# pavlidic/Binary-SpGEMM

Hardware: AMD Instinct MI355X
Metric: output nnz/sec (GNZ/s) (higher is better)
Workload: dtype int32; 1 GPU; R-MAT scale 22, edge factor 16, (a,b,c,d)=(0.30,0.25,0.25,0.20), seed 1, A*A; n=4194304, nnz_a=67108664, products=1336443900, nnz_c=1336366087, parallelism=row-shards x1 cut at equal work, B replicated, priming_steps=0, flow=auto, full=False

## Files before the change

binary-spgemm_amd/bspgemm/__init__.py:

```python
import ctypes as C
import os
import subprocess
import weakref

import numpy as np

os.environ.setdefault("OMP_NUM_THREADS", str(min(16, len(os.sched_getaffinity(0)))))
os.environ.setdefault("GPU_MAX_HW_QUEUES", "8")

_PKG = os.path.dirname(os.path.abspath(__file__))
_ROOT = os.path.dirname(_PKG)
LIB_PATH = os.path.join(_ROOT, "libbspgemm.so")

_I32P = np.ctypeslib.ndpointer(dtype=np.int32, flags="C_CONTIGUOUS")
_I64P = np.ctypeslib.ndpointer(dtype=np.int64, flags="C_CONTIGUOUS")

STATUS = {0: "OK", 1: "ERR_INVALID", 2: "ERR_ALLOC", 3: "ERR_HIP", 4: "ERR_NO_DEVICE",
          5: "ERR_OVERFLOW", 6: "ERR_IO", 7: "ERR_FORMAT", 8: "ERR_COMM", 9: "ERR_SIZE"}

EXPORTS = [
    "bspgemm_status_string", "bspgemm_last_error", "bspgemm_create", "bspgemm_destroy",
    "bspgemm_set_stream", "bspgemm_synchronize", "bspgemm_matrix_upload", "bspgemm_matrix_wrap_device",
    "bspgemm_matrix_free", "bspgemm_matrix_rows", "bspgemm_matrix_cols", "bspgemm_matrix_nnz",
    "bspgemm_multiply", "bspgemm_multiply_masked", "bspgemm_multiply_masked_ex", "bspgemm_result_rows", "bspgemm_result_nnz",
# ... 20 lines not shown
    def __init__(self, status, where=""):
        self.status = status
        msg = lib().bspgemm_last_error().decode(errors="replace") if _lib is not None else ""
        super().__init__("%s: %s %s" % (where, STATUS.get(status, status), msg))


MAX_BINS = 20
FLOWS = {"auto": 0, "upper-bound": 1, "exact": 2}
MASK_COMPLEMENT = 1
CLOSURE_TRANSITIVE = 1
SELECT_OPS = {"tril": 1, "triu": 2, "offdiag": 3}
SETOPS = {"or": 1, "and": 2, "andnot": 3, "xor": 4}
SYMMETRIZE_DROP_DIAGONAL = 1
COMPARES = {">=": 1, ">": 2, "<=": 3, "<": 4, "==": 5, "!=": 6}
OPTIONS = {"class_streams": 1, "blocked_extents": 2, "check": 3, "small_path": 4, "padded_rows": 5,
           "shared_slots": 6}


class Stats(C.Structure):
    _fields_ = [("rows", C.c_int64), ("nnz_a", C.c_int64), ("products", C.c_int64), ("nnz_c", C.c_int64),
                ("bytes_alg", C.c_int64), ("bytes_read_alg", C.c_int64), ("rows_per_bin", C.c_int64 * MAX_BINS),
                ("ms_total", C.c_float), ("ms_symbolic", C.c_float), ("ms_prepass", C.c_float),
                ("ms_count", C.c_float), ("ms_numeric", C.c_float), ("ms_stitch", C.c_float),
                ("ms_bin", C.c_float * MAX_BINS), ("ms_bin_count", C.c_float * MAX_BINS),
                ("t_bin", C.c_float * MAX_BINS), ("t_bin_count", C.c_float * MAX_BINS), ("bins", C.c_int),
                ("bin_cap", C.c_int * MAX_BINS), ("flow", C.c_int), ("prepass_kernel", C.c_int),
                ("class_streams", C.c_int), ("small_path", C.c_int), ("checked", C.c_int), ("padded_rows", C.c_int)]

    def as_dict(self):
        arrays = ("rows_per_bin", "ms_bin", "ms_bin_count", "t_bin", "t_bin_count", "bin_cap")
        d = {k: getattr(self, k) for k, _ in self._fields_ if k not in arrays}
# ... 527 lines not shown
```

binary-spgemm_amd/csrc/context.hip:

```cpp
#include "internal.hpp"

using namespace bsp;

thread_local char bspgemm_err_text[512] = "";

extern "C" const char *bspgemm_last_error(void) { return g_err; }

extern "C" const char *bspgemm_status_string(bspgemm_status s)
{
    switch (s) {
    case BSPGEMM_OK: return "ok";
    case BSPGEMM_ERR_INVALID: return "invalid argument";
    case BSPGEMM_ERR_ALLOC: return "allocation failed";
    case BSPGEMM_ERR_HIP: return "HIP runtime error";
    case BSPGEMM_ERR_NO_DEVICE: return "no gfx950 device (this library has no CPU fallback)";
    case BSPGEMM_ERR_OVERFLOW: return "result exceeds the int32 drop-in interface";
    case BSPGEMM_ERR_IO: return "file I/O error";
    case BSPGEMM_ERR_FORMAT: return "Matrix Market banner rejected";
    case BSPGEMM_ERR_SIZE: return "Matrix Market size line or entry rejected";
    case BSPGEMM_ERR_COMM: return "RCCL error";
    }
    return "unknown status";
}

// ... 121 lines not shown
        for (auto &ph : sl.ev_cls) for (auto &c : ph) for (auto &e : c) HIPCHK_B(hipEventCreate(&e));
    }
    HIPCHK_B(hipStreamCreateWithFlags(&ctx->stream_b, hipStreamNonBlocking));
    HIPCHK_B(hipStreamCreateWithFlags(&ctx->stream_c, hipStreamNonBlocking));
    HIPCHK_B(hipEventCreateWithFlags(&ctx->ev_join, hipEventDisableTiming));
    for (auto &t : ctx->ev_tile) for (auto &e : t) HIPCHK_B(hipEventCreateWithFlags(&e, hipEventDisableTiming));
    ctx->cache_budget = prop.totalGlobalMem / 4;
    if (const char *e = getenv("BSPGEMM_FLOW"))
        ctx->flow = !strcmp(e, "exact") ? BSPGEMM_FLOW_EXACT : (!strcmp(e, "upper-bound") || !strcmp(e, "ub")) ? BSPGEMM_FLOW_UPPER_BOUND : BSPGEMM_FLOW_AUTO;
    if (const char *e = getenv("BSPGEMM_CLASS_TIMING")) ctx->class_timing = atoi(e) != 0;
    if (const char *e = getenv("BSPGEMM_CLASS_STREAMS")) { const int n = atoi(e); ctx->class_streams = n < 1 ? 1 : (n > 3 ? 3 : n); }
    ctx->check = getenv("BSPGEMM_CHECK") != nullptr;
    if (const char *e = getenv("BSPGEMM_RW_BLK")) ctx->rw_blk = atoi(e) ? 1 : 0;
    if (const char *e = getenv("BSPGEMM_SMALL")) ctx->small = atoi(e) ? 1 : 0;
    if (const char *e = getenv("BSPGEMM_PAD_ROWS")) { const int v = atoi(e); ctx->pad_rows = v < 0 ? -1 : (v ? 1 : 0); }
    if (const char *e = getenv("BSPGEMM_SHARED_SLOTS")) { const int v = atoi(e); ctx->shared_slots = v < 0 ? -1 : (v > kSharedSlotsMax ? kSharedSlotsMax : v); }
    ctx->debug_alloc = getenv("BSPGEMM_DEBUG_ALLOC") != nullptr;
    ctx->dropin_timing = getenv("BSPGEMM_DROPIN_TIMING") != nullptr;
    if (ctx->debug_alloc)
        fprintf(stderr, "[bspgemm] device %d: %s, %zu MiB, %d CUs; result cache budget %zu MiB\n", device,
                prop.gcnArchName, (size_t)(prop.totalGlobalMem >> 20), prop.multiProcessorCount, ctx->cache_budget >> 20);
    *out = ctx;
    return BSPGEMM_OK;
}

extern "C" void bspgemm_destroy(bspgemm_context *ctx)
{
    if (!ctx) return;
    hipSetDevice(ctx->device);
    if (ctx->stream) hipStreamSynchronize(ctx->stream);
// ... 379 lines not shown
    case BSPGEMM_OPT_CHECK:
        ctx->check = value != 0;
        return BSPGEMM_OK;
    case BSPGEMM_OPT_SMALL_PATH:
        if (value < -1 || value > 1) return FAIL(BSPGEMM_ERR_INVALID, "small path: -1, 0 or 1");
        ctx->small = value;
        return BSPGEMM_OK;
    case BSPGEMM_OPT_PADDED_ROWS:
        if (value < -1 || value > 1) return FAIL(BSPGEMM_ERR_INVALID, "padded rows: -1, 0 or 1");
        ctx->pad_rows = value;
        return BSPGEMM_OK;
    case BSPGEMM_OPT_SHARED_SLOTS:
        if (value < -1) return FAIL(BSPGEMM_ERR_INVALID, "shared slots: -1, 0 or a count");
        ctx->shared_slots = value > kSharedSlotsMax ? kSharedSlotsMax : value;
        return BSPGEMM_OK;
    }
    return FAIL(BSPGEMM_ERR_INVALID, "unknown option");
}

extern "C" int bspgemm_get_option(const bspgemm_context *ctx, bspgemm_option opt)
{
    if (!ctx) return INT_MIN;
    switch (opt) {
    case BSPGEMM_OPT_CLASS_STREAMS: return ctx->class_streams;
    case BSPGEMM_OPT_BLOCKED_EXTENTS: return ctx->rw_blk;
    case BSPGEMM_OPT_CHECK: return ctx->check ? 1 : 0;
    case BSPGEMM_OPT_SMALL_PATH: return ctx->small;
    case BSPGEMM_OPT_PADDED_ROWS: return ctx->pad_rows;
    case BSPGEMM_OPT_SHARED_SLOTS: return ctx->shared_slots;
    }
    return INT_MIN;
}

extern "C" int bspgemm_matrix_uses_padded_rows(const bspgemm_matrix *m)
{
    if (!m || m->pad_state == 0) return -1;
    return m->pad_state == 1 ? 1 : 0;
}

extern "C" int bspgemm_matrix_uses_blocked_table(const bspgemm_matrix *m)
{
    if (!m || m->blk16_state == 0) return -1;
    return m->blk16_state == 1 ? 1 : 0;
}
// ... 66 lines not shown
```

binary-spgemm_amd/csrc/internal.hpp:

```cpp
#pragma once
#include "../../include/bspgemm.h"
#include "kernels.hpp"

#include <hip/hip_runtime.h>

#include <climits>
#include <cstdio>
#include <cstdlib>
#include <cstring>
#include <chrono>
#include <new>

extern thread_local char bspgemm_err_text[512];
#define g_err bspgemm_err_text

static inline bspgemm_status fail(bspgemm_status st, const char *what, const char *file, int line)
{
    snprintf(g_err, sizeof g_err, "%s (%s:%d)", what, file, line);
    return st;
}
#define FAIL(st, what) fail((st), (what), __FILE__, __LINE__)
#define HIPCHK(call)                                                                       \
    do {                                                                                   \
        hipError_t e_ = (call);                                                            \
// ... 74 lines not shown
    bsp::SmallTiles *d_small_tiles = nullptr;
    unsigned *d_err = nullptr;
    int *chunk_row = nullptr;
    size_t chunk_cap = 0;
    HostScalars *h = nullptr;
    struct CachedBuf { void *p; size_t bytes; };
    CachedBuf cache[8] = {};
    size_t cache_budget = 0;
    int flow = BSPGEMM_FLOW_AUTO;
    bool class_timing = false;
    int class_streams = 2;
    bool check = false;
    int rw_blk = -1;
    int pad_rows = 0;
    int small = -1;
    int shared_slots = -1;
    bool debug_alloc = false;
    bool dropin_timing = false;
};

extern "C" int bspgemm_par_max_plus_one(const int *idx, long long n);
extern "C" void bspgemm_par_prefault(void *p, size_t bytes);
extern "C" long long bspgemm_par_output_bound(const int *Acol, const int *Arow, int r0, int r1, const int *Brow, int brows, long long cap);

struct bspgemm_matrix {
    bspgemm_context *ctx;
    int rows, cols;
    long long nnz;
    int *d_row_ptr, *d_col_idx;
    bool owned;
// ... 42 lines not shown
```

binary-spgemm_amd/csrc/kernels.hpp:

```cpp
#pragma once
#include <hip/hip_runtime.h>
#include <stdint.h>
#include <stdlib.h>

namespace bsp {

enum class MaskMode { None, Keep, Drop, Insert, Count };

constexpr int kWaveBins = 16;
constexpr int kNumBins = kWaveBins + 4;
constexpr int kRankBin = kWaveBins + 1;
constexpr int kMidBin = kWaveBins + 2;
constexpr int kDenseBin = kWaveBins + 3;
constexpr int kRankCap = 6144;
int rank_cap_for_cols(long long cols);
constexpr int kMaxBins = 20;
constexpr int kWaveChunks[kWaveBins + 1] = {0, 1, 2, 3, 4, 5, 6, 7, 8, 10, 12, 14, 16, 20, 24, 28, 32};
constexpr int kMaxWaveCap = 64 * kWaveChunks[kWaveBins];
constexpr int kMidCap = 524288;
inline int mid_cap_for_cols(long long cols)
{
    const long long passes = (cols + (1ll << 18) - 1) >> 18;
    if (passes <= 1) return kMidCap;
    const long long c = kMidCap / passes;
// ... 44 lines not shown
    int bin_count[kNumBins];
    unsigned long long max_f;
};
void launch_scan_and_bin(const long long *F, int n, int row_begin, const int *Arow, long long *prefix,
                         long long *partials, int *bin_tiles, int *bin_count, RowRec *rec,
                         long long *recpre, int *cnt, int heavy_cols, long long *hpartials, int mid_cap, int rank_cap, int bound_cols,
                         hipStream_t s, PrepScalars *scal = nullptr, const long long *true_F = nullptr);

constexpr int kCompactGran = 4096;
inline size_t compact_chunk_rows(long long max_out) { return (size_t)((max_out + kCompactGran - 1) / kCompactGran) + 2; }
void launch_scan_counts(const int *cnt, int n, long long *prefix, long long *partials,
                        const long long *base, hipStream_t s, int *chunk_row = nullptr);

constexpr int kSharedSlotsMax = 16;
int wave_shared_max(int bin, int shared_slots);
constexpr unsigned kErrCapacity = 1u;
constexpr unsigned kErrStaleTable = 2u;
hipError_t launch_wave_rows(int bin, int levels, const int2 *ab, const int *Bcol, int cols,
                            const RowRec *rec, const long long *recpre, const long long *row_ptr, int nrows,
                            int row_begin, int *tmp, int *cnt, unsigned *err, MaskMode mode, const int *Frow, const int *Fcol,
                            hipStream_t s, bool count_only = false, int shared_slots = 0);
void launch_check_tables(const int *row_ptr, int rows, const unsigned char *deg8, const int *blk16, const int *pad_ptr, unsigned *err,
                         hipStream_t s);

void launch_place_heavy(const int *tmp, const RowRec *rec, const long long *recpre, int nrows,
                        const long long *row_ptr, int row_begin, int *col_idx, hipStream_t s);

hipError_t launch_dense_rows(int bin, const int2 *ab, const int *Bcol, long long nnzB, int cols,
                             const RowRec *rec, const long long *recpre, int nrows, int row_begin,
                             int *tmp, int *cnt, MaskMode mode, const int *Frow, const int *Fcol, hipStream_t s,
                             int *vals = nullptr);

constexpr int kHeavySortMax = 8192;
void launch_order_heavy(const RowRec *rec, const long long *recpre, int n, RowRec *rec_out, long long *pre_out, hipStream_t s);

bool wave_masked_supported(int cols);
void launch_wave_masked(int bin, const int2 *ab, const int *Bcol, int cols, const int *Frow, const int *Fcol,
                        const RowRec *rec, const long long *recpre, int nrows, int row_begin,
                        int *tmp, int *cnt, int *vals, hipStream_t s);
hipError_t launch_class(int bin, const int2 *ab, const int *Bcol, long long nnzB, int cols, const RowRec *rec,
                        const long long *recpre, int nrows, int row_begin, int *tmp, int *cnt, unsigned *err, MaskMode mode,
                        const int *Frow, const int *Fcol, hipStream_t s, bool count_only = false, int *vals = nullptr,
                        int shared_slots = 0);
void launch_mask_lengths(const long long *F, const int *Frow, int row_begin, int n, long long *mlen, hipStream_t s);
void launch_mask_lengths_count(const long long *F, const int *Frow, int row_begin, int n, long long *mlen,
                               unsigned long long *maxF, hipStream_t s);
void launch_insert_lengths(const long long *F, const int *Drow, int row_begin, int n, long long *size, hipStream_t s);

void launch_compact(const int *tmp, const long long *Fprefix, const long long *row_ptr,
                    int row_lo, int row_hi, long long max_out, int *col_idx, hipStream_t s, const int *chunk_row = nullptr);

constexpr int kSmallMaxProducts = 65536;
constexpr int kSmallMaxRow = 2048;
constexpr int kSmallMaxRows = 1 << 17;
constexpr int kSmallMaxNnzA = 32768;
struct SmallScalars {
    long long totalF;
    long long nnzC;
// ... 42 lines not shown
```

binary-spgemm_amd/csrc/multiply.hip:

```cpp
#include "internal.hpp"

using namespace bsp;

static bspgemm_status check_operands(bspgemm_context *ctx, const bspgemm_matrix *A, const bspgemm_matrix *B,
                                     int row_begin, int row_end)
{
    if (!ctx || !A || !B) return FAIL(BSPGEMM_ERR_INVALID, "NULL operand");
    if (A->ctx != ctx || B->ctx != ctx) return FAIL(BSPGEMM_ERR_INVALID, "operand belongs to another context");
    if (row_begin < 0 || row_end < row_begin || row_end > A->rows) return FAIL(BSPGEMM_ERR_INVALID, "row range");
    if (B->rows < A->cols) return FAIL(BSPGEMM_ERR_INVALID, "B has fewer rows than A has columns");
    return BSPGEMM_OK;
}


static void class_order(const int *bin_count, long long total_products, int *order, int *lane)
{
    int light[kWaveBins];
    for (int k = 0; k < kWaveBins; k++) light[k] = k + 1;
    const long long heavy_lower_bound = ((long long)bin_count[kRankBin] + bin_count[kMidBin] + bin_count[kDenseBin]) * kMaxWaveCap;
    if (heavy_lower_bound * 8 < total_products) {
        long long key[kNumBins] = {};
        for (int b = 1; b <= kWaveBins; b++) key[b] = (long long)bin_count[b] * kWaveChunks[b];
        for (int a = 1; a < kWaveBins; a++)
            for (int c = a; c > 0 && key[light[c]] > key[light[c - 1]]; c--) {
// ... 204 lines not shown

    if (!ctx->check && result_cached(ctx, result_bytes_colidx(totalF))) {
        HIPCHK_B(alloc_col_idx(ctx, C, totalF));
    } else {
        HIPCHK_B(hipStreamSynchronize(s));
        if (h->nnzC < 0 || h->nnzC > totalF) return bail(FAIL(BSPGEMM_ERR_HIP, "symbolic pass counted more outputs than products"));
        HIPCHK_B(alloc_col_idx(ctx, C, col_cap_for(totalF, h->nnzC)));
    }

    if (R > 0) {
        const int levels = wave_levels_for_cols(B->cols);
        auto emit = [&](int b, int n, const RowRec *rec, const long long *recpre, hipStream_t sx) {
            if (b <= kWaveBins)
                return launch_wave_rows(b, levels, ctx->ab, Bcol, B->cols, rec, recpre, C->d_row_ptr, n, row_begin,
                                        C->d_col_idx, nullptr, ctx->d_err, MaskMode::None, nullptr, nullptr, sx, false,
                                        ctx->shared_slots);
            launch_place_heavy(ctx->tmp, rec, recpre, n, C->d_row_ptr, row_begin, C->d_col_idx, sx);
            return hipSuccess;
        };
        if (bspgemm_status st = class_phase(ctx, 1, totalF, cls_n[1], true, emit)) return bail(st);
    }
    HIPCHK_B(hipEventRecord(slot.ev[3], s));
    if (R > 0) {
        HIPCHK_B(hipEventRecord(ctx->ev_join, ctx->stream_c));
        HIPCHK_B(hipStreamWaitEvent(s, ctx->ev_join, 0));
    }
    return finish_flow(ctx, C, B, totalF, rank_cap_for_cols(B->cols), cls_n, out);
}


static bspgemm_status multiply_upper_bound(bspgemm_context *ctx, const bspgemm_matrix *A,
// ... 40 lines not shown
    if (count && R > 0 && h->prep.max_f > (unsigned long long)INT_MAX)
        return bail(FAIL(BSPGEMM_ERR_OVERFLOW, "a row has more than INT_MAX products: its counts may not fit int32"));
    if (bspgemm_status st = ensure_tmp(ctx, (size_t)total + 1)) return bail(st);
    if (count)
        if (bspgemm_status st = ensure_tmpv(ctx, (size_t)total + 1)) return bail(st);
    if (bspgemm_status st = ensure_chunk_rows(ctx, compact_chunk_rows(total))) return bail(st);
    if (result_cached(ctx, result_bytes_colidx(total))) HIPCHK_B(alloc_col_idx(ctx, C, total));
    HIPCHK_B(hipEventRecord(slot.ev[2], s));

    int cls_n[2][kNumBins] = {};
    if (R > 0) {
        const int *Frow = Fm ? Fm->d_row_ptr : nullptr, *Fcol = Fm ? Fm->d_col_idx : nullptr;
        auto place = [&](int b, int n, const RowRec *rec, const long long *recpre, hipStream_t sx) {
            if (!keep) hub_order(ctx, b, n, rec, recpre, sx);
            return launch_class(b, ctx->ab, Bcol, B->gather_nnz(), B->cols, rec, recpre, n, row_begin, ctx->tmp, ctx->cnt,
                                ctx->d_err, mode, Frow, Fcol, sx, false, count ? ctx->tmpv : nullptr, ctx->shared_slots);
        };
        if (bspgemm_status st = class_phase(ctx, 1, h->products, cls_n[1], false, place)) return bail(st);
        HIPCHK_B(hipEventRecord(slot.ev[3], s));
        launch_scan_counts(ctx->cnt, R, C->d_row_ptr, ctx->partials, nullptr, s, ctx->chunk_row);
    } else {
        HIPCHK_B(hipMemsetAsync(C->d_row_ptr, 0, sizeof(long long), s));
        HIPCHK_B(hipEventRecord(slot.ev[3], s));
    }
    HIPCHK_B(hipMemcpyAsync(&h->nnzC, C->d_row_ptr + R, sizeof(long long), hipMemcpyDeviceToHost, s));
    if (!C->d_col_idx) {
        HIPCHK_B(hipStreamSynchronize(s));
        HIPCHK_B(alloc_col_idx(ctx, C, col_cap_for(total, h->nnzC)));
    }
    if (count)
        HIPCHK_B(result_alloc(ctx, reinterpret_cast<void **>(&C->d_values), result_bytes_colidx(C->col_cap)));
// ... 317 lines not shown
```

binary-spgemm_amd/csrc/wave_rows.hip:

```cpp
#include "kernels.hpp"

namespace bsp {

template <int LEVELS, MaskMode MODE>
void launch_wave_levels(int bin, const int2 *ab, const int *Bcol, int cols, int topw, const RowRec *rec,
                        const long long *recpre, const long long *row_ptr, int nrows, int row_begin, int *tmp, int *cnt,
                        unsigned *err, const int *Frow, const int *Fcol, hipStream_t s, bool count, int shared_max);
#define BSP_WAVE_EXTERN1(L, M) \
    extern template void launch_wave_levels<L, MaskMode::M>(int, const int2 *, const int *, int, int, const RowRec *, \
        const long long *, const long long *, int, int, int *, int *, unsigned *, const int *, const int *, hipStream_t, bool, int);
#define BSP_WAVE_EXTERN(L) BSP_WAVE_EXTERN1(L, None) BSP_WAVE_EXTERN1(L, Drop) BSP_WAVE_EXTERN1(L, Insert)
BSP_WAVE_EXTERN(1) BSP_WAVE_EXTERN(2) BSP_WAVE_EXTERN(3) BSP_WAVE_EXTERN(4) BSP_WAVE_EXTERN(5)
#undef BSP_WAVE_EXTERN
#undef BSP_WAVE_EXTERN1

static int wave_top_words(int levels, int cols)
{
    const long long span = 1ll << (5 * levels);
    return (int)(((long long)cols + span - 1) / span);
}

int wave_shared_max(int bin, int shared_slots)
{
    static_assert(kWaveBins == 16, "one entry per capacity class");
    static const int auto_max[kWaveBins + 1] = {0, 4, 4, 4, 4, 8, 8, 8, 8, 4, 4, 4, 4, 0, 0, 0, 0};
    if (bin < 1 || bin > kWaveBins || kWaveChunks[bin] > 16) return 0;
    if (shared_slots < 0) return auto_max[bin];
    return shared_slots > kSharedSlotsMax ? kSharedSlotsMax : shared_slots;
}

hipError_t launch_wave_rows(int bin, int levels, const int2 *ab, const int *Bcol, int cols,
                            const RowRec *rec, const long long *recpre, const long long *row_ptr, int nrows, int row_begin,
                            int *tmp, int *cnt, unsigned *err, MaskMode mode, const int *Frow, const int *Fcol, hipStream_t s,
                            bool count_only, int shared_slots)
{
    if (mode == MaskMode::Keep || mode == MaskMode::Count || (count_only && mode != MaskMode::None)) return hipErrorInvalidValue;
    if (nrows <= 0) return hipSuccess;
#define BSP_WAVE_ROW(M) {launch_wave_levels<1, MaskMode::M>, launch_wave_levels<2, MaskMode::M>, launch_wave_levels<3, MaskMode::M>, \
                         launch_wave_levels<4, MaskMode::M>, launch_wave_levels<5, MaskMode::M>}
    static const decltype(&launch_wave_levels<1, MaskMode::None>) by_levels[3][5] = {BSP_WAVE_ROW(None), BSP_WAVE_ROW(Drop),
                                                                                      BSP_WAVE_ROW(Insert)};
#undef BSP_WAVE_ROW
    const int m = mode == MaskMode::Drop ? 1 : (mode == MaskMode::Insert ? 2 : 0);
    by_levels[m][(levels < 5 ? levels : 5) - 1](bin, ab, Bcol, cols, wave_top_words(levels, cols), rec, recpre, row_ptr, nrows,
                                                row_begin, tmp, cnt, err, Frow, Fcol, s, count_only,
                                                count_only ? 0 : wave_shared_max(bin, shared_slots));
    return hipSuccess;
}

hipError_t launch_class(int bin, const int2 *ab, const int *Bcol, long long nnzB, int cols, const RowRec *rec,
                        const long long *recpre, int nrows, int row_begin, int *tmp, int *cnt, unsigned *err, MaskMode mode,
                        const int *Frow, const int *Fcol, hipStream_t s, bool count_only, int *vals, int shared_slots)
{
    if (bin > kWaveBins)
        return launch_dense_rows(bin, ab, Bcol, nnzB, cols, rec, recpre, nrows, row_begin, tmp, cnt, mode, Frow, Fcol, s, vals);
    if (mode != MaskMode::Keep && mode != MaskMode::Count)
        return launch_wave_rows(bin, wave_levels_for_cols(cols), ab, Bcol, cols, rec, count_only ? nullptr : recpre, nullptr,
                                nrows, row_begin, count_only ? nullptr : tmp, cnt, err, mode, Frow, Fcol, s, count_only,
                                shared_slots);
    if (!wave_masked_supported(cols))
        return launch_dense_rows(bin, ab, Bcol, nnzB, cols, rec, recpre, nrows, row_begin, tmp, cnt, mode, Frow, Fcol, s, vals);
    launch_wave_masked(bin, ab, Bcol, cols, Frow, Fcol, rec, recpre, nrows, row_begin, tmp, cnt,
                       mode == MaskMode::Count ? vals : nullptr, s);
    return hipSuccess;
}

}
```

binary-spgemm_amd/csrc/wave_rows.inc:

```
#include "kernels.hpp"
#include "wave.hpp"

namespace bsp {

constexpr int waves_per_cu(int w, int bytes) { return (w * bytes > 64 * 1024) ? 0 : (160 * 1024 / (w * bytes)) * w; }

constexpr int prev_wave_chunks(int chunks)
{
    int prev = 0;
    for (int b = 1; b <= kWaveBins; b++) {
        if (kWaveChunks[b] == chunks) return prev;
        prev = kWaveChunks[b];
    }
    return 0;
}

template <int LEVELS, int CHUNKS, int TWP>
struct WaveCfg {
    static constexpr int CAP = 64 * CHUNKS;
    static constexpr int SW = (CHUNKS <= 2) ? CHUNKS : ((CHUNKS + 3) & ~3);
    static constexpr int SLOTS = 64 * SW;
    static constexpr int TOPW = 64 * TWP;
    static constexpr int bytes_per_wave = 4 * TOPW + 2 * TOPW + 8 * CHUNKS + 4 * SLOTS
                                          + (LEVELS >= 2 ? 4 * SLOTS : 16)
                                          + (LEVELS >= 3 ? 4 * SLOTS + 2 * SLOTS : 32)
                                          + (LEVELS >= 4 ? 2 * SLOTS : 16);
    static constexpr int w4 = waves_per_cu(4, bytes_per_wave), w2 = waves_per_cu(2, bytes_per_wave);
    static constexpr int WAVES = (w4 >= w2 && w4 > 0) ? 4 : (w2 > 0 ? 2 : 1);
    static constexpr int RPW = (CHUNKS >= 16) ? kRowsPerWave / 2 : kRowsPerWave;
    static constexpr int FULL = prev_wave_chunks(CHUNKS);
};

template <int CHUNKS, bool SWZ>
__device__ __forceinline__ void store_row(int *out, int n, const u32 *stage, int lane)
{
    const __amdgpu_buffer_rsrc_t rs = __builtin_amdgcn_make_buffer_rsrc((void *)out, (short)0, n * 4, 0x00020000);
#pragma unroll
    for (int c = 0; c < CHUNKS; c++) {
        const int t = c * 64 + lane;
        __builtin_amdgcn_raw_buffer_store_b32(stage[SWZ ? stage_swz(t) : t], rs, t * 4, 0, 2);
    }
}

__device__ __forceinline__ int2 load_extent(const int2 *p)
{
    const long long v = __builtin_nontemporal_load(reinterpret_cast<const long long *>(p));
    return make_int2((int)(u32)v, (int)(u32)((u64)v >> 32));
}

constexpr int kDropBatch = 4;
template <int CHUNKS, bool SWZ>
__device__ __forceinline__ int drop_mask_cols(u32 *stage, int n, u32 *hit, const int *__restrict__ Fcol, int f0, int mlen, int lane)
{
    auto at = [](int p) { return SWZ ? stage_swz(p) : p; };
    const u32 lo = stage[at(0)], hi = stage[at(n - 1)];
// ... 43 lines not shown
        if (keep != valid || kept != c * 64) {
            const u32 v = stage[at(c * 64 + lane)];
            if ((keep >> lane) & 1ull) stage[at(kept + __popcll(keep & mask_lt(lane)))] = v;
        }
        kept += __popcll(keep);
    }
    wave_lds_fence();
    if (lane * 32 < n) hit[lane] = 0u;
    wave_lds_fence();
    return kept;
}

constexpr int kMaxAmbiguous = 12;
constexpr int wr_floor_log2(int x) { int k = 0; while ((2 << k) <= x) k++; return k; }

template <int LEVELS, int CHUNKS, int TWP, MaskMode MODE, bool COUNT>
__global__ __launch_bounds__((64 * WaveCfg<LEVELS, CHUNKS, TWP>::WAVES))
void k_wave_rows(const int2 *__restrict__ ab, const int *__restrict__ Bcol,
                 const RowRec *__restrict__ rec, const long long *__restrict__ recpre,
                 const long long *__restrict__ row_ptr,
                 int nrows, int rpw, int row_begin, int *__restrict__ tmp, int *__restrict__ cnt,
                 unsigned *__restrict__ err, const int *__restrict__ Frow, const int *__restrict__ Fcol, int cols, int shared_max)
{
    constexpr bool EXCL = MODE == MaskMode::Drop, ACC = MODE == MaskMode::Insert;
    constexpr bool FEW = !COUNT && LEVELS >= 2 && CHUNKS <= 16;
    static_assert(!COUNT || MODE == MaskMode::None, "the symbolic pass has no masked form");
    using Cfg = WaveCfg<LEVELS, CHUNKS, TWP>;
    constexpr int TOPW = Cfg::TOPW, WAVES = Cfg::WAVES, SW = Cfg::SW, SLOTS = Cfg::SLOTS, FULL = Cfg::FULL;
    __shared__ __attribute__((aligned(16))) u32 s_top[WAVES][TOPW];
    __shared__ __attribute__((aligned(16))) unsigned short s_topPre[WAVES][TOPW];
    __shared__ __attribute__((aligned(16))) u64 s_starts[WAVES][CHUNKS];
    __shared__ __attribute__((aligned(16))) u32 s_L0w[WAVES][SLOTS];
    __shared__ __attribute__((aligned(16))) u32 s_SA[WAVES][LEVELS >= 2 ? SLOTS : 4];
    __shared__ __attribute__((aligned(16))) u32 s_SB[WAVES][LEVELS >= 3 ? SLOTS : 4];
    __shared__ __attribute__((aligned(16))) unsigned short s_preB[WAVES][LEVELS >= 3 ? SLOTS : 8];
    __shared__ __attribute__((aligned(16))) unsigned short s_preA[WAVES][LEVELS >= 4 ? SLOTS : 8];

    const int lane = lane_id();
    const int plane = (int)(__brev((unsigned)lane) >> 26);
    const int wave_in_wg = threadIdx.x >> 6;
    const long long wave_global = (long long)blockIdx.x * WAVES + wave_in_wg;
    const long long k0 = wave_global * rpw;
    if (k0 >= nrows) return;
    const int nmine = (nrows - k0 < rpw) ? (int)(nrows - k0) : rpw;

    int r_row = 0, r_a0 = 0, r_alen = 0;
    long long r_pre = 0;
    if (lane < nmine) {
        const RowRec q = rec[k0 + lane];
        r_row = q.row;
        r_a0 = q.a0;
        r_alen = q.alen;
        if (!COUNT) r_pre = (EXCL || ACC) ? recpre[k0 + lane] : (row_ptr ? row_ptr[q.row - row_begin] : recpre[k0 + lane]);
    }

    u32 *top = s_top[wave_in_wg];
    unsigned short *topPre = s_topPre[wave_in_wg];
    u64 *starts = s_starts[wave_in_wg];
    u32 *L0w = s_L0w[wave_in_wg];
    int *delta = reinterpret_cast<int *>(s_L0w[wave_in_wg]);
    u32 *SA = s_SA[wave_in_wg];
    u32 *SB = s_SB[wave_in_wg];
    unsigned short *preA = s_preA[wave_in_wg];
    unsigned short *preB = s_preB[wave_in_wg];

    constexpr int TW = TOPW / 64;
    clear_blocked<TW>(top, lane);
    if (lane < CHUNKS) starts[lane] = 0ull;
    if (LEVELS >= 2) clear_blocked<SW>(SA, lane);
    if (LEVELS >= 3) clear_blocked<SW>(SB, lane);
    wave_lds_fence();

    int2 ab_next = make_int2(0, 0);
    {
        const int a0 = wave_bcast(r_a0, 0), alen = wave_bcast(r_alen, 0);
        if (lane < alen) ab_next = load_extent(ab + a0 + lane);
    }
    if (!COUNT) store_row<CHUNKS, false>(tmp, 0, L0w, lane);

    int my_cnt = 0;
    for (int kk = 0; kk < nmine; kk++) {
        const int a0 = wave_bcast(r_a0, kk);
// ... 125 lines not shown
                            }
                            dups += hit != 0ull ? 1 : 0;
                        }
                    }
                }
                running = F - dups;
                row_counted = true;
            }
        }
        if (!row_counted) {
#pragma unroll
        for (int c = 0; c < CHUNKS; c++) {
            {
                if constexpr (ACC) dsrc[c] = dsrc[c] && (u32)col[c] >= (u32)cols;
                const bool ok = ACC ? ((c < FULL || c * 64 + plane < F) && !dsrc[c]) : (c < FULL || c * 64 + plane < F);
                const u32 cc = ok ? (u32)col[c] : 0u;
                col[c] = (int)cc;
                const u32 tw = cc >> (5 * LEVELS);
                if (ok) atomicOr(&top[tw], 1u << ((cc >> (5 * (LEVELS - 1))) & 31));
                rank[c] = (int)tw;
            }
        }
        wave_lds_fence();

        u32 *S0;
        int nslots0 = 0;
        bool few = false;
        int nlose = 0;
        if (LEVELS == 1) {
            S0 = top;
        } else {
            nslots0 = scan_blocked<TW>(top, topPre, lane);
            wave_lds_fence();
            const u32 *P = top;
            const unsigned short *Ppre = topPre;
            u32 *Pmut = top;
            bool parent_is_top = true;
#pragma unroll
            for (int lev = LEVELS - 2; lev >= 0; lev--) {
                const bool sparse = lev == 0 && nslots0 == F;
                if constexpr (FEW) few = lev == 0 && nslots0 != F && F - nslots0 <= shared_max;
                u32 *S = (lev & 1) ? SB : SA;
                unsigned short *Spre = (lev & 1) ? preB : preA;
                u32 px[CHUNKS];
                int ppre[CHUNKS];
#pragma unroll
                for (int c = 0; c < CHUNKS; c++)
                    {
                        px[c] = P[rank[c]];
                        ppre[c] = Ppre[rank[c]];
                    }
#pragma unroll
                for (int c = 0; c < CHUNKS; c++)
                    {
                        const bool ok = ACC ? ((c < FULL || c * 64 + plane < F) && !dsrc[c]) : (c < FULL || c * 64 + plane < F);
                        const u32 cc = (u32)col[c];
// ... 57 lines not shown
                }
#pragma unroll
                for (int c = 0; c < CHUNKS; c++) {
                    const bool ok = ACC ? ((c < FULL || c * 64 + plane < F) && !dsrc[c]) : (c < FULL || c * 64 + plane < F);
                    if (ok) L0w[rank[c]] = (u32)col[c];
                }
                wave_lds_fence();
            }
        }

        constexpr int W0 = (LEVELS == 1) ? TW : SW;
        if (LEVELS >= 2 && (nslots0 == F || few)) {
            running = nslots0 + (few ? nlose : 0);
            if constexpr (EXCL)
                if (running > 0 && mlen > 0) running = drop_mask_cols<CHUNKS, false>(L0w, running, top, Fcol, f0, mlen, lane);
            if (!COUNT) store_row<CHUNKS, false>(out, running, L0w, lane);
        } else if (COUNT) {
            u32 m[W0];
#pragma unroll
            for (int k = 0; k < W0; k++) m[k] = S0[lane * W0 + k];
            clear_blocked<W0>(S0, lane);
            int mine = 0;
#pragma unroll
            for (int k = 0; k < W0; k++) mine += __popc(m[k]);
            running = wave_bcast(wave_incl_scan(mine), 63);
        } else {
            u32 m[W0], wv[W0];
#pragma unroll
            for (int k = 0; k < W0; k++) {
                m[k] = S0[lane * W0 + k];
                wv[k] = (LEVELS == 1) ? (u32)(lane * W0 + k) : (L0w[lane * W0 + k] >> 5);
// ... 10 lines not shown
                int pos = inc - mine;
#pragma unroll
                for (int k = 0; k < W0; k++) {
                    u32 mk = m[k];
                    const u32 base = wv[k] << 5;
                    while (mk) {
                        stage[stage_swz(pos)] = base | (u32)__builtin_ctz(mk);
                        pos++;
                        mk &= mk - 1u;
                    }
                }
            }
            wave_lds_fence();
            if constexpr (EXCL)
                if (running > 0 && mlen > 0) running = drop_mask_cols<CHUNKS, true>(L0w, running, top, Fcol, f0, mlen, lane);
            store_row<CHUNKS, true>(out, running, L0w, lane);
        }
        }
        my_cnt = (lane == kk) ? running : my_cnt;
        wave_lds_fence();
    }
    if (cnt && lane < nmine) cnt[r_row - row_begin] = my_cnt;
}

template <int LEVELS, int CHUNKS, int TWP, MaskMode MODE>
static void launch_cfg(const int2 *ab, const int *Bcol, int cols, const RowRec *rec,
                       const long long *recpre, const long long *row_ptr, int nrows, int row_begin, int *tmp, int *cnt,
                       unsigned *err, hipStream_t s, bool count, const int *Frow, const int *Fcol, int shared_max)
{
    using Cfg = WaveCfg<LEVELS, CHUNKS, TWP>;
    constexpr int kSpreadWaves = 256 * 8;
    int rpw = (int)((nrows + kSpreadWaves - 1) / kSpreadWaves);
    if (rpw > Cfg::RPW) rpw = Cfg::RPW;
    if (rpw < 1) rpw = 1;
    const long long rows_per_wg = (long long)Cfg::WAVES * rpw;
    const int grid = (int)((nrows + rows_per_wg - 1) / rows_per_wg);
    auto kernel = k_wave_rows<LEVELS, CHUNKS, TWP, MODE, false>;
    if constexpr (MODE == MaskMode::None)
        if (count) kernel = k_wave_rows<LEVELS, CHUNKS, TWP, MODE, true>;
    hipLaunchKernelGGL(kernel, dim3(grid), dim3(64 * Cfg::WAVES), 0, s,
                       ab, Bcol, rec, recpre, row_ptr, nrows, rpw, row_begin, tmp, cnt, err, Frow, Fcol, cols, shared_max);
}

template <int LEVELS, int CHUNKS, MaskMode MODE>
static void launch_one(const int2 *ab, const int *Bcol, int cols, int topw, const RowRec *rec,
                       const long long *recpre, const long long *row_ptr, int nrows, int row_begin, int *tmp, int *cnt,
                       unsigned *err, hipStream_t s, bool count, const int *Frow, const int *Fcol, int shared_max)
{
    if (topw <= 128) launch_cfg<LEVELS, CHUNKS, 2, MODE>(ab, Bcol, cols, rec, recpre, row_ptr, nrows, row_begin, tmp, cnt, err, s, count, Frow, Fcol, shared_max);
    else if (topw <= 256) launch_cfg<LEVELS, CHUNKS, 4, MODE>(ab, Bcol, cols, rec, recpre, row_ptr, nrows, row_begin, tmp, cnt, err, s, count, Frow, Fcol, shared_max);
    else if constexpr (LEVELS == 3) launch_cfg<LEVELS, CHUNKS, 8, MODE>(ab, Bcol, cols, rec, recpre, row_ptr, nrows, row_begin, tmp, cnt, err, s, count, Frow, Fcol, shared_max);
}

template <int LEVELS, MaskMode MODE>
void launch_wave_levels(int bin, const int2 *ab, const int *Bcol, int cols, int topw, const RowRec *rec,
                        const long long *recpre, const long long *row_ptr, int nrows, int row_begin, int *tmp, int *cnt,
                        unsigned *err, const int *Frow, const int *Fcol, hipStream_t s, bool count, int shared_max)
{
    switch (bin) {
#define BSP_CASE(b) case b: launch_one<LEVELS, kWaveChunks[b], MODE>(ab, Bcol, cols, topw, rec, recpre, row_ptr, nrows, row_begin, tmp, cnt, err, s, count, Frow, Fcol, shared_max); break;
    BSP_CASE(1) BSP_CASE(2) BSP_CASE(3) BSP_CASE(4) BSP_CASE(5) BSP_CASE(6) BSP_CASE(7) BSP_CASE(8)
    BSP_CASE(9) BSP_CASE(10) BSP_CASE(11) BSP_CASE(12) BSP_CASE(13) BSP_CASE(14) BSP_CASE(15) BSP_CASE(16)
#undef BSP_CASE
    static_assert(kWaveBins == 16, "one case per capacity class");
    default: break;
    }
}

#ifdef BSP_WAVE_LEVELS
template void launch_wave_levels<BSP_WAVE_LEVELS, MaskMode::BSP_WAVE_MODE>(int, const int2 *, const int *, int, int, const RowRec *,
                                                                           const long long *, const long long *, int, int, int *, int *,
                                                                           unsigned *, const int *, const int *, hipStream_t, bool, int);
#endif

}
```

include/bspgemm.h:

```cpp
#ifndef BSPGEMM_H
#define BSPGEMM_H

#include <stddef.h>
#include <stdint.h>

#ifdef __cplusplus
extern "C" {
#endif

typedef enum bspgemm_status {
    BSPGEMM_OK            = 0,
    BSPGEMM_ERR_INVALID   = 1,
    BSPGEMM_ERR_ALLOC     = 2,
    BSPGEMM_ERR_HIP       = 3,
    BSPGEMM_ERR_NO_DEVICE = 4,
    BSPGEMM_ERR_OVERFLOW  = 5,
    BSPGEMM_ERR_IO        = 6,
    BSPGEMM_ERR_FORMAT    = 7,
    BSPGEMM_ERR_COMM      = 8,
    BSPGEMM_ERR_SIZE      = 9
} bspgemm_status;

const char *bspgemm_status_string(bspgemm_status s);
const char *bspgemm_last_error(void);
// ... 29 lines not shown
                                int row_begin, int row_end, bspgemm_result **C);

#define BSPGEMM_FLOW_AUTO        0
#define BSPGEMM_FLOW_UPPER_BOUND 1
#define BSPGEMM_FLOW_EXACT       2
bspgemm_status bspgemm_set_flow(bspgemm_context *ctx, int flow);

bspgemm_status bspgemm_set_class_timing(bspgemm_context *ctx, int on);

typedef enum bspgemm_option {
    BSPGEMM_OPT_CLASS_STREAMS   = 1,
    BSPGEMM_OPT_BLOCKED_EXTENTS = 2,
    BSPGEMM_OPT_CHECK           = 3,
    BSPGEMM_OPT_SMALL_PATH      = 4,
    BSPGEMM_OPT_PADDED_ROWS     = 5,
    BSPGEMM_OPT_SHARED_SLOTS    = 6
} bspgemm_option;
bspgemm_status bspgemm_set_option(bspgemm_context *ctx, bspgemm_option opt, int value);
int            bspgemm_get_option(const bspgemm_context *ctx, bspgemm_option opt);
int            bspgemm_matrix_uses_blocked_table(const bspgemm_matrix *m);
int            bspgemm_matrix_uses_padded_rows(const bspgemm_matrix *m);

bspgemm_status bspgemm_multiply_masked(bspgemm_context *ctx,
                                       const bspgemm_matrix *A, const bspgemm_matrix *B,
                                       const bspgemm_matrix *F,
                                       int row_begin, int row_end, bspgemm_result **C);

#define BSPGEMM_MASK_COMPLEMENT 1u
bspgemm_status bspgemm_multiply_masked_ex(bspgemm_context *ctx,
                                          const bspgemm_matrix *A, const bspgemm_matrix *B,
                                          const bspgemm_matrix *F, unsigned flags,
// ... 173 lines not shown
```

Baseline: 239.3 GNZ/s.

## Left-shift column ids into the wide top bitmap and alias top buffers into level scratch

```diff
diff --git a/binary-spgemm_amd/bspgemm/__init__.py b/binary-spgemm_amd/bspgemm/__init__.py
--- a/binary-spgemm_amd/bspgemm/__init__.py
+++ b/binary-spgemm_amd/bspgemm/__init__.py
@@ -58,7 +58,7 @@
 SYMMETRIZE_DROP_DIAGONAL = 1
 COMPARES = {">=": 1, ">": 2, "<=": 3, "<": 4, "==": 5, "!=": 6}
 OPTIONS = {"class_streams": 1, "blocked_extents": 2, "check": 3, "small_path": 4, "padded_rows": 5,
-           "shared_slots": 6}
+           "shared_slots": 6, "scaled_columns": 7}
 
 
 class Stats(C.Structure):
diff --git a/binary-spgemm_amd/csrc/context.hip b/binary-spgemm_amd/csrc/context.hip
--- a/binary-spgemm_amd/csrc/context.hip
+++ b/binary-spgemm_amd/csrc/context.hip
@@ -159,6 +159,7 @@
     if (const char *e = getenv("BSPGEMM_RW_BLK")) ctx->rw_blk = atoi(e) ? 1 : 0;
     if (const char *e = getenv("BSPGEMM_SMALL")) ctx->small = atoi(e) ? 1 : 0;
     if (const char *e = getenv("BSPGEMM_PAD_ROWS")) { const int v = atoi(e); ctx->pad_rows = v < 0 ? -1 : (v ? 1 : 0); }
+    if (const char *e = getenv("BSPGEMM_SCALED_COLUMNS")) ctx->scaled_columns = atoi(e) != 0;
     if (const char *e = getenv("BSPGEMM_SHARED_SLOTS")) { const int v = atoi(e); ctx->shared_slots = v < 0 ? -1 : (v > kSharedSlotsMax ? kSharedSlotsMax : v); }
     ctx->debug_alloc = getenv("BSPGEMM_DEBUG_ALLOC") != nullptr;
     ctx->dropin_timing = getenv("BSPGEMM_DROPIN_TIMING") != nullptr;
@@ -568,6 +569,10 @@
         if (value < -1) return FAIL(BSPGEMM_ERR_INVALID, "shared slots: -1, 0 or a count");
         ctx->shared_slots = value > kSharedSlotsMax ? kSharedSlotsMax : value;
         return BSPGEMM_OK;
+    case BSPGEMM_OPT_SCALED_COLUMNS:
+        if (value < 0 || value > 1) return FAIL(BSPGEMM_ERR_INVALID, "scaled columns: 0 or 1");
+        ctx->scaled_columns = value;
+        return BSPGEMM_OK;
     }
     return FAIL(BSPGEMM_ERR_INVALID, "unknown option");
 }
@@ -582,6 +587,7 @@
     case BSPGEMM_OPT_SMALL_PATH: return ctx->small;
     case BSPGEMM_OPT_PADDED_ROWS: return ctx->pad_rows;
     case BSPGEMM_OPT_SHARED_SLOTS: return ctx->shared_slots;
+    case BSPGEMM_OPT_SCALED_COLUMNS: return ctx->scaled_columns;
     }
     return INT_MIN;
 }
diff --git a/binary-spgemm_amd/csrc/internal.hpp b/binary-spgemm_amd/csrc/internal.hpp
--- a/binary-spgemm_amd/csrc/internal.hpp
+++ b/binary-spgemm_amd/csrc/internal.hpp
@@ -112,6 +112,7 @@
     int rw_blk = -1;
     int pad_rows = 0;
     int small = -1;
+    int scaled_columns = 1;
     int shared_slots = -1;
     bool debug_alloc = false;
     bool dropin_timing = false;
diff --git a/binary-spgemm_amd/csrc/kernels.hpp b/binary-spgemm_amd/csrc/kernels.hpp
--- a/binary-spgemm_amd/csrc/kernels.hpp
+++ b/binary-spgemm_amd/csrc/kernels.hpp
@@ -82,12 +82,20 @@
 
 constexpr int kSharedSlotsMax = 16;
 int wave_shared_max(int bin, int shared_slots);
+constexpr bool wave_scaled_chunks(int chunks) { return chunks >= 10 && chunks <= 16; }
+bool wave_scaled_class(int bin, int scaled_columns);
+inline int wave_col_shift(int64_t cols)
+{
+    int sh = 0;
+    while (sh < 5 && (cols << (sh + 1)) <= ((int64_t)kWaveTopWordsWide << 15)) sh++;
+    return sh;
+}
 constexpr unsigned kErrCapacity = 1u;
 constexpr unsigned kErrStaleTable = 2u;
 hipError_t launch_wave_rows(int bin, int levels, const int2 *ab, const int *Bcol, int cols,
                             const RowRec *rec, const long long *recpre, const long long *row_ptr, int nrows,
                             int row_begin, int *tmp, int *cnt, unsigned *err, MaskMode mode, const int *Frow, const int *Fcol,
-                            hipStream_t s, bool count_only = false, int shared_slots = 0);
+                            hipStream_t s, bool count_only = false, int shared_slots = 0, int scaled_columns = 0);
 void launch_check_tables(const int *row_ptr, int rows, const unsigned char *deg8, const int *blk16, const int *pad_ptr, unsigned *err,
                          hipStream_t s);
 
@@ -109,7 +117,7 @@
 hipError_t launch_class(int bin, const int2 *ab, const int *Bcol, long long nnzB, int cols, const RowRec *rec,
                         const long long *recpre, int nrows, int row_begin, int *tmp, int *cnt, unsigned *err, MaskMode mode,
                         const int *Frow, const int *Fcol, hipStream_t s, bool count_only = false, int *vals = nullptr,
-                        int shared_slots = 0);
+                        int shared_slots = 0, int scaled_columns = 0);
 void launch_mask_lengths(const long long *F, const int *Frow, int row_begin, int n, long long *mlen, hipStream_t s);
 void launch_mask_lengths_count(const long long *F, const int *Frow, int row_begin, int n, long long *mlen,
                                unsigned long long *maxF, hipStream_t s);
diff --git a/binary-spgemm_amd/csrc/multiply.hip b/binary-spgemm_amd/csrc/multiply.hip
--- a/binary-spgemm_amd/csrc/multiply.hip
+++ b/binary-spgemm_amd/csrc/multiply.hip
@@ -242,7 +242,7 @@
             if (b <= kWaveBins)
                 return launch_wave_rows(b, levels, ctx->ab, Bcol, B->cols, rec, recpre, C->d_row_ptr, n, row_begin,
                                         C->d_col_idx, nullptr, ctx->d_err, MaskMode::None, nullptr, nullptr, sx, false,
-                                        ctx->shared_slots);
+                                        ctx->shared_slots, ctx->scaled_columns);
             launch_place_heavy(ctx->tmp, rec, recpre, n, C->d_row_ptr, row_begin, C->d_col_idx, sx);
             return hipSuccess;
         };
@@ -313,7 +313,7 @@
         auto place = [&](int b, int n, const RowRec *rec, const long long *recpre, hipStream_t sx) {
             if (!keep) hub_order(ctx, b, n, rec, recpre, sx);
             return launch_class(b, ctx->ab, Bcol, B->gather_nnz(), B->cols, rec, recpre, n, row_begin, ctx->tmp, ctx->cnt,
-                                ctx->d_err, mode, Frow, Fcol, sx, false, count ? ctx->tmpv : nullptr, ctx->shared_slots);
+                                ctx->d_err, mode, Frow, Fcol, sx, false, count ? ctx->tmpv : nullptr, ctx->shared_slots, ctx->scaled_columns);
         };
         if (bspgemm_status st = class_phase(ctx, 1, h->products, cls_n[1], false, place)) return bail(st);
         HIPCHK_B(hipEventRecord(slot.ev[3], s));
diff --git a/binary-spgemm_amd/csrc/wave_rows.hip b/binary-spgemm_amd/csrc/wave_rows.hip
--- a/binary-spgemm_amd/csrc/wave_rows.hip
+++ b/binary-spgemm_amd/csrc/wave_rows.hip
@@ -5,10 +5,10 @@
 template <int LEVELS, MaskMode MODE>
 void launch_wave_levels(int bin, const int2 *ab, const int *Bcol, int cols, int topw, const RowRec *rec,
                         const long long *recpre, const long long *row_ptr, int nrows, int row_begin, int *tmp, int *cnt,
-                        unsigned *err, const int *Frow, const int *Fcol, hipStream_t s, bool count, int shared_max);
+                        unsigned *err, const int *Frow, const int *Fcol, hipStream_t s, bool count, int shared_max, bool scaled);
 #define BSP_WAVE_EXTERN1(L, M) \
     extern template void launch_wave_levels<L, MaskMode::M>(int, const int2 *, const int *, int, int, const RowRec *, \
-        const long long *, const long long *, int, int, int *, int *, unsigned *, const int *, const int *, hipStream_t, bool, int);
+        const long long *, const long long *, int, int, int *, int *, unsigned *, const int *, const int *, hipStream_t, bool, int, bool);
 #define BSP_WAVE_EXTERN(L) BSP_WAVE_EXTERN1(L, None) BSP_WAVE_EXTERN1(L, Drop) BSP_WAVE_EXTERN1(L, Insert)
 BSP_WAVE_EXTERN(1) BSP_WAVE_EXTERN(2) BSP_WAVE_EXTERN(3) BSP_WAVE_EXTERN(4) BSP_WAVE_EXTERN(5)
 #undef BSP_WAVE_EXTERN
@@ -29,10 +29,15 @@
     return shared_slots > kSharedSlotsMax ? kSharedSlotsMax : shared_slots;
 }
 
+bool wave_scaled_class(int bin, int scaled_columns)
+{
+    return scaled_columns != 0 && bin >= 1 && bin <= kWaveBins && wave_scaled_chunks(kWaveChunks[bin]);
+}
+
 hipError_t launch_wave_rows(int bin, int levels, const int2 *ab, const int *Bcol, int cols,
                             const RowRec *rec, const long long *recpre, const long long *row_ptr, int nrows, int row_begin,
                             int *tmp, int *cnt, unsigned *err, MaskMode mode, const int *Frow, const int *Fcol, hipStream_t s,
-                            bool count_only, int shared_slots)
+                            bool count_only, int shared_slots, int scaled_columns)
 {
     if (mode == MaskMode::Keep || mode == MaskMode::Count || (count_only && mode != MaskMode::None)) return hipErrorInvalidValue;
     if (nrows <= 0) return hipSuccess;
@@ -44,20 +49,21 @@
     const int m = mode == MaskMode::Drop ? 1 : (mode == MaskMode::Insert ? 2 : 0);
     by_levels[m][(levels < 5 ? levels : 5) - 1](bin, ab, Bcol, cols, wave_top_words(levels, cols), rec, recpre, row_ptr, nrows,
                                                 row_begin, tmp, cnt, err, Frow, Fcol, s, count_only,
-                                                count_only ? 0 : wave_shared_max(bin, shared_slots));
+                                                count_only ? 0 : wave_shared_max(bin, shared_slots),
+                                                !count_only && wave_scaled_class(bin, scaled_columns));
     return hipSuccess;
 }
 
 hipError_t launch_class(int bin, const int2 *ab, const int *Bcol, long long nnzB, int cols, const RowRec *rec,
                         const long long *recpre, int nrows, int row_begin, int *tmp, int *cnt, unsigned *err, MaskMode mode,
-                        const int *Frow, const int *Fcol, hipStream_t s, bool count_only, int *vals, int shared_slots)
+                        const int *Frow, const int *Fcol, hipStream_t s, bool count_only, int *vals, int shared_slots, int scaled_columns)
 {
     if (bin > kWaveBins)
         return launch_dense_rows(bin, ab, Bcol, nnzB, cols, rec, recpre, nrows, row_begin, tmp, cnt, mode, Frow, Fcol, s, vals);
     if (mode != MaskMode::Keep && mode != MaskMode::Count)
         return launch_wave_rows(bin, wave_levels_for_cols(cols), ab, Bcol, cols, rec, count_only ? nullptr : recpre, nullptr,
                                 nrows, row_begin, count_only ? nullptr : tmp, cnt, err, mode, Frow, Fcol, s, count_only,
-                                shared_slots);
+                                shared_slots, scaled_columns);
     if (!wave_masked_supported(cols))
         return launch_dense_rows(bin, ab, Bcol, nnzB, cols, rec, recpre, nrows, row_begin, tmp, cnt, mode, Frow, Fcol, s, vals);
     launch_wave_masked(bin, ab, Bcol, cols, Frow, Fcol, rec, recpre, nrows, row_begin, tmp, cnt,
diff --git a/binary-spgemm_amd/csrc/wave_rows.inc b/binary-spgemm_amd/csrc/wave_rows.inc
--- a/binary-spgemm_amd/csrc/wave_rows.inc
+++ b/binary-spgemm_amd/csrc/wave_rows.inc
@@ -15,13 +15,14 @@
     return 0;
 }
 
-template <int LEVELS, int CHUNKS, int TWP>
+template <int LEVELS, int CHUNKS, int TWP, bool ALIAS = false>
 struct WaveCfg {
     static constexpr int CAP = 64 * CHUNKS;
     static constexpr int SW = (CHUNKS <= 2) ? CHUNKS : ((CHUNKS + 3) & ~3);
     static constexpr int SLOTS = 64 * SW;
     static constexpr int TOPW = 64 * TWP;
-    static constexpr int bytes_per_wave = 4 * TOPW + 2 * TOPW + 8 * CHUNKS + 4 * SLOTS
+    static_assert(!ALIAS || (LEVELS == 3 && SLOTS >= TOPW), "top and topPre must fit into SA and preB");
+    static constexpr int bytes_per_wave = (ALIAS ? 32 : 4 * TOPW + 2 * TOPW) + 8 * CHUNKS + 4 * SLOTS
                                           + (LEVELS >= 2 ? 4 * SLOTS : 16)
                                           + (LEVELS >= 3 ? 4 * SLOTS + 2 * SLOTS : 32)
                                           + (LEVELS >= 4 ? 2 * SLOTS : 16);
@@ -31,14 +32,15 @@
     static constexpr int FULL = prev_wave_chunks(CHUNKS);
 };
 
-template <int CHUNKS, bool SWZ>
-__device__ __forceinline__ void store_row(int *out, int n, const u32 *stage, int lane)
+template <int CHUNKS, bool SWZ, bool SCALED = false>
+__device__ __forceinline__ void store_row(int *out, int n, const u32 *stage, int lane, int sh = 0)
 {
     const __amdgpu_buffer_rsrc_t rs = __builtin_amdgcn_make_buffer_rsrc((void *)out, (short)0, n * 4, 0x00020000);
 #pragma unroll
     for (int c = 0; c < CHUNKS; c++) {
         const int t = c * 64 + lane;
-        __builtin_amdgcn_raw_buffer_store_b32(stage[SWZ ? stage_swz(t) : t], rs, t * 4, 0, 2);
+        const u32 v = stage[SWZ ? stage_swz(t) : t];
+        __builtin_amdgcn_raw_buffer_store_b32(SCALED ? v >> sh : v, rs, t * 4, 0, 2);
     }
 }
 
@@ -112,8 +114,10 @@
 constexpr int kMaxAmbiguous = 12;
 constexpr int wr_floor_log2(int x) { int k = 0; while ((2 << k) <= x) k++; return k; }
 
-template <int LEVELS, int CHUNKS, int TWP, MaskMode MODE, bool COUNT>
-__global__ __launch_bounds__((64 * WaveCfg<LEVELS, CHUNKS, TWP>::WAVES))
+constexpr bool wave_top_alias(bool sc, int chunks, int twp) { return sc && (chunks <= 2 ? chunks : ((chunks + 3) & ~3)) >= twp; }
+
+template <int LEVELS, int CHUNKS, int TWP, MaskMode MODE, bool COUNT, bool SC = false>
+__global__ __launch_bounds__((64 * WaveCfg<LEVELS, CHUNKS, TWP, wave_top_alias(SC, CHUNKS, TWP)>::WAVES))
 void k_wave_rows(const int2 *__restrict__ ab, const int *__restrict__ Bcol,
                  const RowRec *__restrict__ rec, const long long *__restrict__ recpre,
                  const long long *__restrict__ row_ptr,
@@ -123,10 +127,14 @@
     constexpr bool EXCL = MODE == MaskMode::Drop, ACC = MODE == MaskMode::Insert;
     constexpr bool FEW = !COUNT && LEVELS >= 2 && CHUNKS <= 16;
     static_assert(!COUNT || MODE == MaskMode::None, "the symbolic pass has no masked form");
-    using Cfg = WaveCfg<LEVELS, CHUNKS, TWP>;
+    static_assert(!SC || (!COUNT && LEVELS == 3 && MODE == MaskMode::None), "scaled columns: the emitting three-level instances only");
+    constexpr bool ALIAS = wave_top_alias(SC, CHUNKS, TWP);
+    using Cfg = WaveCfg<LEVELS, CHUNKS, TWP, ALIAS>;
+    const int sh = SC ? shared_max >> 8 : 0;
+    const int few_max = SC ? shared_max & 255 : shared_max;
     constexpr int TOPW = Cfg::TOPW, WAVES = Cfg::WAVES, SW = Cfg::SW, SLOTS = Cfg::SLOTS, FULL = Cfg::FULL;
-    __shared__ __attribute__((aligned(16))) u32 s_top[WAVES][TOPW];
-    __shared__ __attribute__((aligned(16))) unsigned short s_topPre[WAVES][TOPW];
+    __shared__ __attribute__((aligned(16))) u32 s_top[WAVES][ALIAS ? 4 : TOPW];
+    __shared__ __attribute__((aligned(16))) unsigned short s_topPre[WAVES][ALIAS ? 8 : TOPW];
     __shared__ __attribute__((aligned(16))) u64 s_starts[WAVES][CHUNKS];
     __shared__ __attribute__((aligned(16))) u32 s_L0w[WAVES][SLOTS];
     __shared__ __attribute__((aligned(16))) u32 s_SA[WAVES][LEVELS >= 2 ? SLOTS : 4];
@@ -152,8 +160,8 @@
         if (!COUNT) r_pre = (EXCL || ACC) ? recpre[k0 + lane] : (row_ptr ? row_ptr[q.row - row_begin] : recpre[k0 + lane]);
     }
 
-    u32 *top = s_top[wave_in_wg];
-    unsigned short *topPre = s_topPre[wave_in_wg];
+    u32 *top = ALIAS ? s_SA[wave_in_wg] : s_top[wave_in_wg];
+    unsigned short *topPre = ALIAS ? s_preB[wave_in_wg] : s_topPre[wave_in_wg];
     u64 *starts = s_starts[wave_in_wg];
     u32 *L0w = s_L0w[wave_in_wg];
     int *delta = reinterpret_cast<int *>(s_L0w[wave_in_wg]);
@@ -163,7 +171,7 @@
     unsigned short *preB = s_preB[wave_in_wg];
 
     constexpr int TW = TOPW / 64;
-    clear_blocked<TW>(top, lane);
+    if (!ALIAS) clear_blocked<TW>(top, lane);
     if (lane < CHUNKS) starts[lane] = 0ull;
     if (LEVELS >= 2) clear_blocked<SW>(SA, lane);
     if (LEVELS >= 3) clear_blocked<SW>(SB, lane);
@@ -319,7 +327,7 @@
             {
                 if constexpr (ACC) dsrc[c] = dsrc[c] && (u32)col[c] >= (u32)cols;
                 const bool ok = ACC ? ((c < FULL || c * 64 + plane < F) && !dsrc[c]) : (c < FULL || c * 64 + plane < F);
-                const u32 cc = ok ? (u32)col[c] : 0u;
+                const u32 cc = ok ? (SC ? (u32)col[c] << sh : (u32)col[c]) : 0u;
                 col[c] = (int)cc;
                 const u32 tw = cc >> (5 * LEVELS);
                 if (ok) atomicOr(&top[tw], 1u << ((cc >> (5 * (LEVELS - 1))) & 31));
@@ -344,7 +352,7 @@
 #pragma unroll
             for (int lev = LEVELS - 2; lev >= 0; lev--) {
                 const bool sparse = lev == 0 && nslots0 == F;
-                if constexpr (FEW) few = lev == 0 && nslots0 != F && F - nslots0 <= shared_max;
+                if constexpr (FEW) few = lev == 0 && nslots0 != F && F - nslots0 <= few_max;
                 u32 *S = (lev & 1) ? SB : SA;
                 unsigned short *Spre = (lev & 1) ? preB : preA;
                 u32 px[CHUNKS];
@@ -432,7 +440,7 @@
             running = nslots0 + (few ? nlose : 0);
             if constexpr (EXCL)
                 if (running > 0 && mlen > 0) running = drop_mask_cols<CHUNKS, false>(L0w, running, top, Fcol, f0, mlen, lane);
-            if (!COUNT) store_row<CHUNKS, false>(out, running, L0w, lane);
+            if (!COUNT) store_row<CHUNKS, false, SC>(out, running, L0w, lane, sh);
         } else if (COUNT) {
             u32 m[W0];
 #pragma unroll
@@ -473,7 +481,7 @@
             wave_lds_fence();
             if constexpr (EXCL)
                 if (running > 0 && mlen > 0) running = drop_mask_cols<CHUNKS, true>(L0w, running, top, Fcol, f0, mlen, lane);
-            store_row<CHUNKS, true>(out, running, L0w, lane);
+            store_row<CHUNKS, true, SC>(out, running, L0w, lane, sh);
         }
         }
         my_cnt = (lane == kk) ? running : my_cnt;
@@ -482,20 +490,20 @@
     if (cnt && lane < nmine) cnt[r_row - row_begin] = my_cnt;
 }
 
-template <int LEVELS, int CHUNKS, int TWP, MaskMode MODE>
+template <int LEVELS, int CHUNKS, int TWP, MaskMode MODE, bool SC = false>
 static void launch_cfg(const int2 *ab, const int *Bcol, int cols, const RowRec *rec,
                        const long long *recpre, const long long *row_ptr, int nrows, int row_begin, int *tmp, int *cnt,
                        unsigned *err, hipStream_t s, bool count, const int *Frow, const int *Fcol, int shared_max)
 {
-    using Cfg = WaveCfg<LEVELS, CHUNKS, TWP>;
+    using Cfg = WaveCfg<LEVELS, CHUNKS, TWP, wave_top_alias(SC, CHUNKS, TWP)>;
     constexpr int kSpreadWaves = 256 * 8;
     int rpw = (int)((nrows + kSpreadWaves - 1) / kSpreadWaves);
     if (rpw > Cfg::RPW) rpw = Cfg::RPW;
     if (rpw < 1) rpw = 1;
     const long long rows_per_wg = (long long)Cfg::WAVES * rpw;
     const int grid = (int)((nrows + rows_per_wg - 1) / rows_per_wg);
-    auto kernel = k_wave_rows<LEVELS, CHUNKS, TWP, MODE, false>;
-    if constexpr (MODE == MaskMode::None)
+    auto kernel = k_wave_rows<LEVELS, CHUNKS, TWP, MODE, false, SC>;
+    if constexpr (MODE == MaskMode::None && !SC)
         if (count) kernel = k_wave_rows<LEVELS, CHUNKS, TWP, MODE, true>;
     hipLaunchKernelGGL(kernel, dim3(grid), dim3(64 * Cfg::WAVES), 0, s,
                        ab, Bcol, rec, recpre, row_ptr, nrows, rpw, row_begin, tmp, cnt, err, Frow, Fcol, cols, shared_max);
@@ -504,8 +512,15 @@
 template <int LEVELS, int CHUNKS, MaskMode MODE>
 static void launch_one(const int2 *ab, const int *Bcol, int cols, int topw, const RowRec *rec,
                        const long long *recpre, const long long *row_ptr, int nrows, int row_begin, int *tmp, int *cnt,
-                       unsigned *err, hipStream_t s, bool count, const int *Frow, const int *Fcol, int shared_max)
-{
+                       unsigned *err, hipStream_t s, bool count, const int *Frow, const int *Fcol, int shared_max, bool scaled)
+{
+    if constexpr (LEVELS == 3 && MODE == MaskMode::None && wave_scaled_chunks(CHUNKS)) {
+        if (scaled && !count) {
+            launch_cfg<LEVELS, CHUNKS, kWaveTopWordsWide / 64, MODE, true>(ab, Bcol, cols, rec, recpre, row_ptr, nrows, row_begin, tmp, cnt, err, s, false,
+                                                                          Frow, Fcol, (shared_max & 255) | (wave_col_shift(cols) << 8));
+            return;
+        }
+    }
     if (topw <= 128) launch_cfg<LEVELS, CHUNKS, 2, MODE>(ab, Bcol, cols, rec, recpre, row_ptr, nrows, row_begin, tmp, cnt, err, s, count, Frow, Fcol, shared_max);
     else if (topw <= 256) launch_cfg<LEVELS, CHUNKS, 4, MODE>(ab, Bcol, cols, rec, recpre, row_ptr, nrows, row_begin, tmp, cnt, err, s, count, Frow, Fcol, shared_max);
     else if constexpr (LEVELS == 3) launch_cfg<LEVELS, CHUNKS, 8, MODE>(ab, Bcol, cols, rec, recpre, row_ptr, nrows, row_begin, tmp, cnt, err, s, count, Frow, Fcol, shared_max);
@@ -514,10 +529,10 @@
 template <int LEVELS, MaskMode MODE>
 void launch_wave_levels(int bin, const int2 *ab, const int *Bcol, int cols, int topw, const RowRec *rec,
                         const long long *recpre, const long long *row_ptr, int nrows, int row_begin, int *tmp, int *cnt,
-                        unsigned *err, const int *Frow, const int *Fcol, hipStream_t s, bool count, int shared_max)
+                        unsigned *err, const int *Frow, const int *Fcol, hipStream_t s, bool count, int shared_max, bool scaled)
 {
     switch (bin) {
-#define BSP_CASE(b) case b: launch_one<LEVELS, kWaveChunks[b], MODE>(ab, Bcol, cols, topw, rec, recpre, row_ptr, nrows, row_begin, tmp, cnt, err, s, count, Frow, Fcol, shared_max); break;
+#define BSP_CASE(b) case b: launch_one<LEVELS, kWaveChunks[b], MODE>(ab, Bcol, cols, topw, rec, recpre, row_ptr, nrows, row_begin, tmp, cnt, err, s, count, Frow, Fcol, shared_max, scaled); break;
     BSP_CASE(1) BSP_CASE(2) BSP_CASE(3) BSP_CASE(4) BSP_CASE(5) BSP_CASE(6) BSP_CASE(7) BSP_CASE(8)
     BSP_CASE(9) BSP_CASE(10) BSP_CASE(11) BSP_CASE(12) BSP_CASE(13) BSP_CASE(14) BSP_CASE(15) BSP_CASE(16)
 #undef BSP_CASE
@@ -529,7 +544,7 @@
 #ifdef BSP_WAVE_LEVELS
 template void launch_wave_levels<BSP_WAVE_LEVELS, MaskMode::BSP_WAVE_MODE>(int, const int2 *, const int *, int, int, const RowRec *,
                                                                            const long long *, const long long *, int, int, int *, int *,
-                                                                           unsigned *, const int *, const int *, hipStream_t, bool, int);
+                                                                           unsigned *, const int *, const int *, hipStream_t, bool, int, bool);
 #endif
 
 }
diff --git a/include/bspgemm.h b/include/bspgemm.h
--- a/include/bspgemm.h
+++ b/include/bspgemm.h
@@ -67,7 +67,8 @@
     BSPGEMM_OPT_CHECK           = 3,
     BSPGEMM_OPT_SMALL_PATH      = 4,
     BSPGEMM_OPT_PADDED_ROWS     = 5,
-    BSPGEMM_OPT_SHARED_SLOTS    = 6
+    BSPGEMM_OPT_SHARED_SLOTS    = 6,
+    BSPGEMM_OPT_SCALED_COLUMNS  = 7
 } bspgemm_option;
 bspgemm_status bspgemm_set_option(bspgemm_context *ctx, bspgemm_option opt, int value);
 int            bspgemm_get_option(const bspgemm_context *ctx, bspgemm_option opt);
```

Result: no change. 241.3 GNZ/s, median of 6 (+0.9%).
